# z430/keyword-spotting

Hardware: AMD Instinct MI355X
Metric: 1s 16kHz clips/sec end-to-end (wav->label) (higher is better)
Workload: dtype f32

## Files before the change

### keyword-spotting_amd/csrc/kws_dscnn.hip

```cpp
#include <array>
#include <utility>

#include "kws_dscnn_stages.h"

namespace kws {
namespace {

#ifndef KWS_X_DSCNN_STAMP_TID
#define KWS_X_DSCNN_STAMP_TID 0
#endif

__device__ __forceinline__ DscnnWeights weights_for_this_clip() {
#if defined(__HIP_DEVICE_COMPILE__)
    using KArg = const __attribute__((address_space(4))) DscnnWeights*;
    KArg p = (KArg)__builtin_amdgcn_kernarg_segment_ptr();
    asm volatile("" : "+s"(p));
    return *p;
#else
    return DscnnWeights{};
#endif
}

using FwdKernelFn = void (*)(DscnnWeights, const float*, int, float*, int32_t*, float*, unsigned long long*, const int*, StreamPush);
struct FwdKernelArgs {
// ... 134 lines not shown

    constexpr bool SPLIT = MODE >= 4;
    constexpr bool UT = PERSIST && PAIR;
    BlockTables t1p{};
    uintx4 c1p[PERSIST ? 7 : 1][NP];
    int prev_clip = -1;
    float* a_prev = nullptr;
    if ((MODE == 4 || MODE == 5) && !CLUSTER && tid_k == 0) lds[OFF_ARRIVE] = 0.f;
    if constexpr (PERSIST) {
        fetch_block_tables(w_arg, 1, tid_k, t1p);
        if (wv_k < STAGE_WAVES) stage_features_persist<PAIR, SCAN>(lds, feat, clip, tid_k, sp.scan);
        load_conv1_frags(w_arg, wv_k, lane_k, c1p);
        __syncthreads();
    }
    for (;;) {
    auto weights_now = [&]() -> DscnnWeights { return PERSIST ? weights_for_this_clip() : w_arg; };
    const DscnnWeights w = weights_now();
    int tid = tid_k;
    if constexpr (PERSIST) {
        int wv_l = __builtin_amdgcn_readfirstlane(wv_k), lane_l = lane_k;
        asm volatile("" : "+s"(wv_l), "+v"(lane_l));
        tid = (wv_l << 6) | (lane_l & 63);
    }
    const int lane = tid & 63, wv = tid >> 6;
    if constexpr (PERSIST) n_stamp = 0;
    if (stamps && tid == KWS_X_DSCNN_STAMP_TID) stamps[(size_t)clip * KWS_DSCNN_STAMPS + KWS_DSCNN_STAMPS - 2] = __builtin_amdgcn_s_memrealtime();
    stamp();

    PwOperands<MODE> wa;
    UnitDesc ud{};
    int hops_before = 0;
    int kx = 0, ky[5] = {0, 0, 0, 0, 0}, sg[5] = {0, 0, 0, 0, 0};
    if constexpr (PERSIST) {
        if constexpr (PAIR) {
            const float mxf = read_stage_max(lds, 0, 1);
            kx = pow2_exp_for(mxf);
            const float bz0 = (w.c1_abs * mxf + w.c1_bmax) * 1.001f;
            cap_units(kx, sg[0], w.k_c1, bz0);
            const float by1 = (w.dw_abs[0] * bz0 + w.dw_bmax[0]) * 1.001f;
            ky[1] = pow2_exp_for(by1);
            cap_units(ky[1], sg[1], w.k_pw[0], (w.pw_abs[0] * by1 + w.pw_bmax[0]) * 1.001f);
            store_block_tables(lds, 1, tid, t1p, pow2f(ky[1]), pow2f(sg[1]), pow2f(ky[1] - sg[0]));
            conv1_build_windows(lds, tid, pow2f(kx), OFF_FEAT_P);
            __syncthreads();
        } else {
            store_block_tables(lds, 1, tid, t1p);
        }
        stamp();
        conv1_phase_split<false, NP>(w, lds, tid, c1p, rg0, pow2f(kx), pow2f(sg[0]), OFF_FEAT_P);
        if (wv == NW - 1 && prev_clip >= 0) {
            pool_fc_wave(w, lds, lane, prev_clip, logits, label, a_prev);
            if (stamps && lane == 0) stamps[(size_t)prev_clip * KWS_DSCNN_STAMPS + 13] = __builtin_amdgcn_s_memtime();
        }
        if constexpr (UT) load_unit_desc(w, 1, wv < Leftover<1>::TILE ? wv : Leftover<1>::TILE, lane, ud);
        load_afrag(w, 1, wv >= 4 ? wv - 4 : 0, lane, wa.ring[0]);
    } else if constexpr (PRECONV) {
        static_assert(!PRECONV || MODE >= 4, "the pre-convolved entry exists for the product (split) path only");
        const float* z = feat + (size_t)clip * (CH * P0);
        fetch_block_tables(w, 1, tid, t1_pre);
        float zmax = 0.f;
        for (int i = tid; i < CH * P0; i += NT) {
            const float v = z[i];
            lds[OFF_Z0 + pidx(i / P0, i % P0, P0 + 2)] = v;
            zmax = fmaxf(zmax, v);
        }
        if (tid < CH) {
            lds[OFF_Z0 + pidx(tid, P0, P0 + 2)] = 0.f;
            lds[OFF_Z0 + pidx(tid, P0 + 1, P0 + 2)] = 0.f;
        }
        if constexpr (PAIR)
            publish_wave_max(lds, 1, wv, lane, zmax);
        else
            store_block_tables(lds, 1, tid, t1_pre);
        if constexpr (Leftover<1>::HAS && (MODE == 4 || MODE == 5) && !CLUSTER)
            load_afrag(w, 1, wv >= 4 ? wv - 4 : 0, lane, wa.ring[0]);
        else
            load_block_head(w, 1, lane, wa);
        stamp();
    } else {
    float* featp = lds + OFF_FEAT;
    const float* f = clip_features<SCAN>(feat, clip, sp.scan);
    constexpr int FV = (IN_T * IN_F + NT - 1) / NT;
    float fv[FV];
    int row_new = -1;
    int head;
    if constexpr (STREAM) {
        hops_before = *sp.hops;
        const int K = frames_lag(sp.p);
        head = (((hops_before + 2 - K) % IN_T) + IN_T) % IN_T;
        const int step = sp.p.frame_step;
        const long f_start = (long)step * hops_before + step - (long)K * step;
        if (f_start >= 0) row_new = (int)((((f_start / step) - head) % IN_T + IN_T) % IN_T);
    } else {
        head = ring_hops ? (((*ring_hops + 1 - sp.frames_lag) % IN_T) + IN_T) % IN_T : 0;
    }
#pragma unroll
    for (int k = 0; k < FV; ++k) {
        const int i = tid + k * NT;
        fv[k] = (i < IN_T * IN_F && i / IN_F != row_new) ? f[((i / IN_F + head) % IN_T) * IN_F + i % IN_F] : 0.f;
    }
    BlockTables t1;
    fetch_block_tables(w, 1, tid, t1);
    __builtin_amdgcn_sched_barrier(0);
    float a1[SPLIT ? 1 : 50];
    uintx4 c1f[SPLIT ? 7 : 1][NP];
    if constexpr (SPLIT) {
        load_conv1_frags(w, wv, lane, c1f);
    } else if constexpr (MFMA) {
        const int half = lane >> 5, col = lane & 31, ct = wv & 1;
#pragma unroll
        for (int s = 0; s < 50; ++s) a1[s] = w.c1_w[(2 * s + half) * CH + ct * 32 + col];
        load_pointwise(w, 1, lane, wa);
    }
    __builtin_amdgcn_sched_barrier(0);
    if constexpr (PAIR) {
        float m = 0.f;
#pragma unroll
        for (int k = 0; k < FV; ++k) m = fmaxf(m, fabsf(fv[k]));
        publish_wave_max(lds, 0, wv, lane, m);
    }
    if constexpr (STREAM) {
#ifdef KWS_X_STREAM_NO_FRAME
        if (false)
#else
        if (wv == 0 && cl_tile == cl_n - 1)
#endif
            stream_frame_wave(sp.p, sp.t, sp.hop, clip, clip, false, sp.pcm_ring, sp.ring_len, const_cast<float*>(feat), hops_before,
                              reinterpret_cast<unsigned char*>(lds + OFF_Z2), lane,
                              row_new >= 0 ? featp + (row_new + 2) * FEAT_W + 2 : nullptr, sp.refine_ctr);
        for (int i = tid; i < FEAT_H * FEAT_W; i += NT) {
            const int r = i / FEAT_W - 2, c = i % FEAT_W - 2;
            if (!((unsigned)r < (unsigned)IN_T && (unsigned)c < (unsigned)IN_F)) featp[i] = 0.f;
        }
        if constexpr (!PAIR) store_block_tables(lds, 1, tid, t1);
#pragma unroll
        for (int k = 0; k < FV; ++k) {
            const int i = tid + k * NT;
            if (i < IN_T * IN_F && i / IN_F != row_new) featp[(i / IN_F + 2) * FEAT_W + (i % IN_F) + 2] = fv[k];
        }
        __syncthreads();
    } else {
    for (int i = tid; i < FEAT_H * FEAT_W; i += NT) {
        const int r = i / FEAT_W - 2, c = i % FEAT_W - 2;
        if (!((unsigned)r < (unsigned)IN_T && (unsigned)c < (unsigned)IN_F)) featp[i] = 0.f;
    }
    if constexpr (!PAIR) store_block_tables(lds, 1, tid, t1);
#pragma unroll
    for (int k = 0; k < FV; ++k) {
        const int i = tid + k * NT;
        if (i < IN_T * IN_F) featp[(i / IN_F + 2) * FEAT_W + (i % IN_F) + 2] = fv[k];
    }
    __syncthreads();
    }
    if constexpr (PAIR) {
        float mxf = read_stage_max(lds, 0, 1);
        if constexpr (STREAM) {
            if (row_new >= 0 && cl_tile == cl_n - 1)
                for (int c = 0; c < IN_F; ++c) mxf = fmaxf(mxf, fabsf(featp[(row_new + 2) * FEAT_W + 2 + c]));
        }
        kx = pow2_exp_for(mxf);
        const float bz0 = (w.c1_abs * mxf + w.c1_bmax) * 1.001f;
        cap_units(kx, sg[0], w.k_c1, bz0);
        const float by1 = (w.dw_abs[0] * bz0 + w.dw_bmax[0]) * 1.001f;
        ky[1] = pow2_exp_for(by1);
        cap_units(ky[1], sg[1], w.k_pw[0], (w.pw_abs[0] * by1 + w.pw_bmax[0]) * 1.001f);
        store_block_tables(lds, 1, tid, t1, pow2f(ky[1]), pow2f(sg[1]), pow2f(ky[1] - sg[0]));
        conv1_build_windows(lds, tid, pow2f(kx));
        __syncthreads();
    }
    stamp();

    if constexpr (SPLIT) {
        conv1_phase_split<CLUSTER, NP>(w, lds, tid, c1f, rg0, pow2f(kx), pow2f(sg[0]));
        if constexpr (Leftover<1>::HAS && (MODE == 4 || MODE == 5) && !CLUSTER)
            load_afrag(w, 1, wv >= 4 ? wv - 4 : 0, lane, wa.ring[0]);
        else
            load_block_head(w, 1, lane, wa);
    } else {
        conv1_phase<MFMA>(w, lds, tid, a1);
    }
    }
    stamp();
    const DscnnWeights w1 = weights_now();
    __syncthreads();
    stamp();
    float* a = act ? act + (size_t)clip * KWS_ACT_FLOATS_PER_CLIP : nullptr;
    if (a) {
        const float u = PAIR ? pow2f(-sg[0]) : 1.f;
        for (int i = tid; i < CH * P0; i += NT) a[i] = lds[OFF_Z0 + pidx(i / P0, i % P0, P0 + 2)] * u;
        a += CH * P0;
    }
    PairCtx pc;
    if constexpr (PAIR && PRECONV) {
        const float mz0 = read_stage_max(lds, 1, 1);
        const float by1 = (w1.dw_abs[0] * mz0 + w1.dw_bmax[0]) * 1.001f;
        ky[1] = pow2_exp_for(by1);
        cap_units(ky[1], sg[1], w1.k_pw[0], (w1.pw_abs[0] * by1 + w1.pw_bmax[0]) * 1.001f);
        store_block_tables(lds, 1, tid, t1_pre, pow2f(ky[1]), pow2f(sg[1]), pow2f(ky[1]));
        __syncthreads();
    }
    if constexpr (PAIR) {
        const float mz = read_stage_max(lds, 1, 1) * pow2f(-sg[0]);
        const float bz = (w1.pw_abs[0] * ((w1.dw_abs[0] * mz + w1.dw_bmax[0]) * 1.001f) + w1.pw_bmax[0]) * 1.001f;
        const float by = (w1.dw_abs[1] * bz + w1.dw_bmax[1]) * 1.001f;
        ky[2] = pow2_exp_for(by);
        cap_units(ky[2], sg[2], w1.k_pw[1], (w1.pw_abs[1] * by + w1.pw_bmax[1]) * 1.001f);
        pc.s_dww = pow2f(ky[2] - sg[1]);
        pc.s_dwb = pow2f(ky[2]);
        pc.s_pwb = pow2f(sg[2]);
    }
    block_phase<1, MODE, CLUSTER, UT>(w1, lds, tid, wa, ud, nullptr, rg1, pc);
    stamp();
    const DscnnWeights w2 = weights_now();
    __syncthreads();
    stamp();
    if (a) {
        const float u = PAIR ? pow2f(-sg[1]) : 1.f;
        for (int i = tid; i < CH * Blk<1>::POUT; i += NT)
            a[i] = lds[OFF_Z1 + pidx(i / Blk<1>::POUT, i % Blk<1>::POUT, Blk<1>::SOUT)] * u;
        a += CH * Blk<1>::POUT;
    }
    if constexpr (PAIR) {
        const float mz = fmaxf(read_stage_max(lds, 2, 1) * pow2f(-sg[1]), w2.pw_bmax[0]);
        const float bz = (w2.pw_abs[1] * ((w2.dw_abs[1] * mz + w2.dw_bmax[1]) * 1.001f) + w2.pw_bmax[1]) * 1.001f;
        const float by = (w2.dw_abs[2] * bz + w2.dw_bmax[2]) * 1.001f;
        ky[3] = pow2_exp_for(by);
        cap_units(ky[3], sg[3], w2.k_pw[2], (w2.pw_abs[2] * by + w2.pw_bmax[2]) * 1.001f);
        pc.s_dww = pow2f(ky[3] - sg[2]);
// ... 261 lines not shown
```

### keyword-spotting_amd/csrc/kws_dscnn_geom.h

```cpp
#pragma once
#include "kws_internal.h"

namespace kws {
namespace {

#ifndef KWS_DSCNN_WAVES
#define KWS_DSCNN_WAVES 8
#endif
constexpr int NW = KWS_DSCNN_WAVES;
constexpr int NT = NW * 64;
constexpr int TW = 30;

constexpr int P0 = C1_H * C1_W;
constexpr int FEAT_H = 103, FEAT_W = 14;
constexpr int OFF_Z3 = 0, OFF_Z2 = 22976, OFF_Z1 = 0, OFF_Z0 = 9152, OFF_FEAT = 18304;
constexpr int OFF_DWTAB = 38784;
constexpr int OFF_PWB = OFF_DWTAB + 2 * 768;
constexpr int OFF_POOLED = OFF_PWB + 2 * 64;
constexpr int OFF_POOLBUF = OFF_DWTAB;
constexpr int OFF_WMAX = OFF_POOLED + 64 + 8;
constexpr int OFF_ARRIVE = OFF_WMAX + 3 * NW;
constexpr int LDS_FLOATS = 40960;
static_assert(OFF_ARRIVE + 1 <= LDS_FLOATS, "LDS overflow");
static_assert(NW * 64 <= 768, "pool scratch must fit one depthwise buffer");
static_assert(OFF_FEAT + FEAT_H * FEAT_W <= OFF_Z2, "feature pad overlaps Z2");
static_assert(CH * 12 <= 2 * NT, "table staging assumes at most two elements per thread");

__host__ __device__ __forceinline__ constexpr int pidx(int c, int p, int S) { return (c >> 1) * 2 * S + 2 * p + (c & 1); }

template <int N>
struct Blk {
    static constexpr int H = 45 + 2 * N, W = 1 + 2 * N;
    static constexpr bool RING = N > 1;
    static constexpr int HI = RING ? H - 2 : H, WI = RING ? W - 2 : W;
    static constexpr int PIN = HI * WI, SIN = PIN + 2;
    static constexpr int POUT = H * W, SOUT = POUT + 2;
    static constexpr int OFF_IN = N == 1 ? OFF_Z0 : N == 2 ? OFF_Z1 : N == 3 ? OFF_Z2 : OFF_Z3;
    static constexpr int OFF_OUT = N == 1 ? OFF_Z1 : N == 2 ? OFF_Z2 : OFF_Z3;
    static constexpr int TILES = (POUT + TW - 1) / TW;
    static constexpr int BUF = (N - 1) & 1;
};

#ifndef KWS_DSCNN_KSPLIT_LEFTOVER
#define KWS_DSCNN_KSPLIT_LEFTOVER 1
#endif
template <int N>
struct Leftover {
    static constexpr bool HAS = KWS_DSCNN_KSPLIT_LEFTOVER && (N == 1 || N == 2);
    static constexpr int TILE = N == 1 ? 4 : 8;
    static constexpr int P0T = TILE * TW;
    static constexpr int NP = HAS ? Blk<N>::POUT - P0T : 1;
    static constexpr int WAVE0 = N == 1 ? 4 : 0;
    static constexpr int OFF_PART = N == 1 ? OFF_Z2 : OFF_Z0;
    static constexpr int CSTRIDE = CH + 4;
    static constexpr int PART = NP * CSTRIDE;
};
static_assert(Blk<1>::TILES == 5 && Blk<2>::TILES == 9, "the leftover tiles are the fifth of block 1 and the ninth of block 2");
static_assert(4 * Leftover<1>::PART <= 38784 - OFF_Z2 && OFF_Z0 + 4 * Leftover<2>::PART <= OFF_FEAT, "partial sums fit their dead planes");
static_assert(Leftover<1>::OFF_PART % 4 == 0 && Leftover<2>::OFF_PART % 4 == 0 && Leftover<1>::CSTRIDE % 4 == 0, "partial sums move as float4s");

constexpr int OFF_FEAT_P = OFF_Z2;
constexpr int OFF_POOLBUF_P = OFF_FEAT_P + 1456;
constexpr int STAGE_WAVES = 4;
static_assert(OFF_FEAT_P >= OFF_Z3 + Blk<3>::SOUT * CH, "the next clip's features must not overlap block 4's input");
static_assert(OFF_FEAT_P + FEAT_H * FEAT_W <= OFF_POOLBUF_P && OFF_POOLBUF_P % 4 == 0, "features and pool partials are disjoint");
static_assert(OFF_POOLBUF_P + NW * CH <= OFF_Z2 + Blk<2>::SOUT * CH && OFF_Z2 + Blk<2>::SOUT * CH <= OFF_DWTAB,
              "pool partials stay inside the Z2 plane, clear of the table buffers the next clip's block 1 rewrites");

}
}
```

### keyword-spotting_amd/csrc/kws_dscnn_stages.h

```cpp
#pragma once
#include <type_traits>

#include "kws_dscnn_geom.h"
#include "kws_dscnn_units.h"
#include "kws_mfcc_dev.h"
#include "kws_split_mfma.h"

namespace kws {
namespace {

template <bool TO_MFMA = false>
__device__ __forceinline__ float stencil3x3(float w0, float w1, float w2, float w3, float w4, float w5, float w6,
                                            float w7, float w8, float b, float up, float mid, float dn, float mask_l,
                                            float mask_r) {
    float c, to_right, to_left;
    asm("v_mul_f32 %1, %3, %13\n\t"
        "v_mul_f32 %2, %5, %13\n\t"
        "v_fma_f32 %0, %4, %13, %12\n\t"
        "v_fmac_f32 %1, %6, %14\n\t"
        "v_fmac_f32 %2, %8, %14\n\t"
        "v_fmac_f32 %0, %7, %14\n\t"
        "v_fmac_f32 %1, %9, %15\n\t"
        "v_fmac_f32 %2, %11, %15\n\t"
        "v_fmac_f32 %0, %10, %15\n\t"
// ... 68 lines not shown
    mx = step(mx, std::integral_constant<int, 0x114>{}, std::integral_constant<int, 0xf>{});
    mx = step(mx, std::integral_constant<int, 0x118>{}, std::integral_constant<int, 0xf>{});
    mx = step(mx, std::integral_constant<int, 0x142>{}, std::integral_constant<int, 0xa>{});
    mx = step(mx, std::integral_constant<int, 0x143>{}, std::integral_constant<int, 0xc>{});
    if (lane == 63) lds[OFF_WMAX + set * NW + wv] = mx;
}
__device__ __forceinline__ float read_stage_max(const float* lds, int set0, int n_sets) {
    static_assert(NW % 4 == 0 && OFF_WMAX % 4 == 0, "the stage maxima are read as float4s");
    float m = 0.f;
    const float4* q = reinterpret_cast<const float4*>(lds + OFF_WMAX + set0 * NW);
    for (int i = 0; i < (NW / 4) * n_sets; ++i) {
        const float4 v = q[i];
        m = fmaxf(fmaxf(m, fmaxf(v.x, v.y)), fmaxf(v.z, v.w));
    }
    return m;
}

template <int NP>
struct PwRing {
    uintx4 ring[2][2][NP];
};
struct PwRegsF32 {
    float wa[2][32];
};
template <int MODE>
using PwOperands = std::conditional_t<(MODE >= 4), PwRing<(MODE == 5 ? 2 : 3)>, PwRegsF32>;
__device__ __forceinline__ void load_pointwise(const DscnnWeights& w, int n, int lane, PwRegsF32& o) {
    const float* pw = w.pw_w + (n - 1) * CH * CH + 8 * (lane >> 5) * CH + (lane & 31);
#pragma unroll
    for (int ct = 0; ct < 2; ++ct)
#pragma unroll
        for (int s = 0; s < 32; ++s) o.wa[ct][s] = pw[(16 * (s >> 3) + (s & 7)) * CH + ct * 32];
}
template <int NP>
__device__ __forceinline__ void load_afrag(const DscnnWeights& w, int n, int m, int lane, uintx4 (&f)[2][NP]) {
    const uintx4* src = reinterpret_cast<const uintx4*>(NP == 2 ? w.pw_pair : w.pw_split) + (size_t)(n - 1) * (2 * 4 * NP * 64) + lane;
#pragma unroll
    for (int ct = 0; ct < 2; ++ct)
#pragma unroll
        for (int p = 0; p < NP; ++p) f[ct][p] = src[((ct * 4 + m) * NP + p) * 64];
}
__device__ __forceinline__ void load_block_head(const DscnnWeights& w, int n, int lane, PwRegsF32& o) { load_pointwise(w, n, lane, o); }
template <int NP>
__device__ __forceinline__ void load_block_head(const DscnnWeights& w, int n, int lane, PwRing<NP>& o) { load_afrag(w, n, 0, lane, o.ring[0]); }

struct UnitDesc {
    uintx4 a;
    uint2 m;
};
__device__ __forceinline__ void load_unit_desc(const DscnnWeights& w, int n, int tile, int lane, UnitDesc& d) {
    const uint32_t* src = w.units + ((size_t)(ds_unit_base(n - 1) + tile) * 2 * 64 + lane) * 4;
    d.a = *reinterpret_cast<const uintx4*>(src);
    d.m = *reinterpret_cast<const uint2*>(src + 64 * 4);
}

template <bool MFMA>
__device__ __forceinline__ void conv1_phase(const DscnnWeights& w, float* lds, int tid, const float (&a)[50]) {
    const float* featp = lds + OFF_FEAT;
    float* z0 = lds + OFF_Z0;
    if constexpr (MFMA) {
        const int lane = tid & 63, wv = tid >> 6, half = lane >> 5, col = lane & 31;
        const int ct = wv & 1;
        for (int u = wv; u < 10; u += NW) {
            const int pt = u >> 1;
            const int pos = pt * 32 + col;
            const int posc = pos < P0 ? pos : P0 - 1;
            const int oh = posc / C1_W, ow = posc % C1_W;
            const float* base = featp + (2 * oh) * FEAT_W + 2 * ow + half;
            floatx16 acc = {0, 0, 0, 0, 0, 0, 0, 0, 0, 0, 0, 0, 0, 0, 0, 0};
#pragma unroll
            for (int s = 0; s < 50; ++s) {
                const float b = base[((2 * s) / 10) * FEAT_W + (2 * s) % 10];
                acc = __builtin_amdgcn_mfma_f32_32x32x2f32(a[s], b, acc, 0, 0, 0);
            }
            if (pos < P0) {
#pragma unroll
                for (int r = 0; r < 16; ++r) {
                    const int co = ct * 32 + row_of(r, half);
                    z0[pidx(co, pos, P0 + 2)] = relu(acc[r] + w.c1_b[co]);
                }
            }
        }
    } else {
        for (int idx = tid; idx < CH * P0; idx += NT) {
            const int co = idx / P0, pos = idx % P0;
            const int oh = pos / C1_W, ow = pos % C1_W;
            float acc = w.c1_b[co];
            for (int kh = 0; kh < C1_K; ++kh)
                for (int kw = 0; kw < C1_K; ++kw)
                    acc = fmaf(w.c1_w[(kh * C1_K + kw) * CH + co], featp[(2 * oh + kh) * FEAT_W + 2 * ow + kw], acc);
            z0[pidx(co, pos, P0 + 2)] = relu(acc);
        }
    }
    if (tid < CH) {
        z0[pidx(tid, P0, P0 + 2)] = 0.f;
        z0[pidx(tid, P0 + 1, P0 + 2)] = 0.f;
    }
}

template <bool DUAL, int NP>
__device__ __forceinline__ void conv1_unit_split(const DscnnWeights& w, const float* featp, float* z0, int ptile, int ct, int lane,
                                                 const uintx4 (&c1f)[7][NP], int p_lo, int p_hi, float sx, float sig0, float& mx) {
    constexpr bool PAIR = NP == 2;
    const int half = lane >> 5, col = lane & 31;
    const int pos = p_lo + ptile * 32 + col;
    const int posc = pos < p_hi ? pos : p_hi - 1;
// ... 210 lines not shown
        for (int r = 0; r < 16; r += 2) {
            const int co = ct * 32 + row_of(r, half);
            const float4 b4 = cb[r >> 2];
            const float b0 = (r & 2) ? b4.z : b4.x, b1 = (r & 2) ? b4.w : b4.y;
            const float v0 = relu(fmaf(b0, sig0, acc[r])), v1 = relu(fmaf(b1, sig0, acc[r + 1]));
            *reinterpret_cast<float2*>(z0 + pidx(co, pos, P0 + 2)) = make_float2(v0, v1);
            mx = fmaxf(mx, fmaxf(v0, v1));
            if (DUAL) {
                const int oo = (ct ^ 1) * 32 + row_of(r, half);
                const float4 o4 = ob[DUAL ? (r >> 2) : 0];
                const float c0 = (r & 2) ? o4.z : o4.x, c1 = (r & 2) ? o4.w : o4.y;
                const float u0 = relu(fmaf(c0, sig0, occ[r])), u1 = relu(fmaf(c1, sig0, occ[r + 1]));
                *reinterpret_cast<float2*>(z0 + pidx(oo, pos, P0 + 2)) = make_float2(u0, u1);
                mx = fmaxf(mx, fmaxf(u0, u1));
            }
        }
    }
}

struct PosRange {
    int lo, hi;
};

template <bool RANGED, int NP>
__device__ __forceinline__ void conv1_phase_split(const DscnnWeights& w, float* lds, int tid, const uintx4 (&c1f)[7][NP],
                                                  PosRange rg, float sx = 1.f, float sig0 = 1.f, int off_feat = OFF_FEAT) {
    static_assert(P0 > 4 * 32 && P0 <= 5 * 32 && NW >= 6, "conv1 work split: four dual tiles + one tile in two halves");
    const float* featp = lds + off_feat;
    float* z0 = lds + OFF_Z0;
    const int lane = tid & 63, wv = tid >> 6;
    float mx = 0.f;
    if constexpr (NP == 2) {
        if constexpr (RANGED) {
            const int n_pt = (rg.hi - rg.lo + 31) / 32;
            for (int u = wv; u < 2 * n_pt; u += NW) conv1_unit_pairwin<false>(w, lds, z0, u >> 1, u & 1, lane, c1f, rg.lo, rg.hi, sig0, mx);
        } else if (wv < 4)
            conv1_unit_pairwin<true>(w, lds, z0, wv, wv & 1, lane, c1f, 0, P0, sig0, mx);
        else if (wv < 6)
            conv1_unit_pairwin<false>(w, lds, z0, 4, wv & 1, lane, c1f, 0, P0, sig0, mx);
    } else if constexpr (RANGED) {
        const int n_pt = (rg.hi - rg.lo + 31) / 32;
        for (int u = wv; u < 2 * n_pt; u += NW) conv1_unit_split<false, NP>(w, featp, z0, u >> 1, u & 1, lane, c1f, rg.lo, rg.hi, sx, sig0, mx);
    } else if (wv < 4)
        conv1_unit_split<true, NP>(w, featp, z0, wv, wv & 1, lane, c1f, 0, P0, sx, sig0, mx);
    else if (wv < 6)
        conv1_unit_split<false, NP>(w, featp, z0, 4, wv & 1, lane, c1f, 0, P0, sx, sig0, mx);
    if constexpr (NP == 2) publish_wave_max(lds, 1, wv, lane, mx);
    if (tid < CH) {
        z0[pidx(tid, P0, P0 + 2)] = 0.f;
        z0[pidx(tid, P0 + 1, P0 + 2)] = 0.f;
    }
}

template <int N, int NP, bool UT = false>
__device__ __forceinline__ void leftover_partial_unit(float* lds, int lane, int M, const uintx4 (&af)[2][NP], const UnitDesc& ud) {
    using G = Blk<N>;
    using L = Leftover<N>;
    const int half = lane >> 5, col = lane & 31;
    const float* dwtab = lds + OFF_DWTAB + G::BUF * 768;
    const float4* dwt4 = reinterpret_cast<const float4*>(dwtab) + half * 24;
    bool valid;
    float mask_l, mask_r;
    int ta[3];
    if constexpr (UT) {
        valid = ud.a[3] != 0u;
        mask_l = __builtin_bit_cast(float, ud.m.x), mask_r = __builtin_bit_cast(float, ud.m.y);
#pragma unroll
        for (int i = 0; i < 3; ++i) ta[i] = (int)ud.a[i];
    } else {
        const int pos = L::P0T - 1 + col;
        valid = col >= 1 && col <= TW && pos < G::POUT;
        const int posc = pos < G::POUT ? pos : G::POUT - 1;
        const int h = posc / G::W, x = posc % G::W;
        mask_l = x > 0 ? 1.f : 0.f, mask_r = x < G::W - 1 ? 1.f : 0.f;
#pragma unroll
        for (int dh = -1; dh <= 1; ++dh) {
            const int o = G::RING ? 1 : 0;
            const int hh = h + dh - o, xx = x - o;
            const bool inside = (unsigned)hh < (unsigned)G::HI && (unsigned)xx < (unsigned)G::WI;
            const bool in_map = (unsigned)(h + dh) < (unsigned)G::H;
            const int a = inside ? hh * G::WI + xx : ((G::RING && in_map) ? G::PIN : G::PIN + 1);
            ta[dh + 1] = G::OFF_IN + pidx(half * 8, a, G::SIN);
        }
    }
    float y[8];
#pragma unroll
    for (int j = 0; j < 8; j += 2) {
        const int cs = 16 * M + j;
        const int o = cs * G::SIN;
        const float2 up = *reinterpret_cast<const float2*>(lds + ta[0] + o);
        const float2 mid = *reinterpret_cast<const float2*>(lds + ta[1] + o);
        const float2 dn = *reinterpret_cast<const float2*>(lds + ta[2] + o);
        DwPair wp;
#pragma unroll
        for (int i = 0; i < 5; ++i) wp.l[i] = dwt4[(cs >> 1) * 6 + i];
        y[j] = stencil3x3_of_pair<false, 0>(wp, up.x, mid.x, dn.x, mask_l, mask_r);
        y[j + 1] = stencil3x3_of_pair<false, 1>(wp, up.y, mid.y, dn.y, mask_l, mask_r);
    }
    floatx16 acc0 = {0, 0, 0, 0, 0, 0, 0, 0, 0, 0, 0, 0, 0, 0, 0, 0}, acc1 = acc0;
    if constexpr (NP == 2) {
        uintx4 bh, bl;
        split_pair8_scaled(y, bh, bl);
        acc0 = mfma_f16(af[0][0], bl, acc0);
        acc1 = mfma_f16(af[1][0], bl, acc1);
        acc0 = mfma_f16(af[0][1], bh, acc0);
        acc1 = mfma_f16(af[1][1], bh, acc1);
        acc0 = mfma_f16(af[0][0], bh, acc0);
        acc1 = mfma_f16(af[1][0], bh, acc1);
    } else {
        uintx4 bh, bm, bl;
        split3(y, bh, bm, bl);
#pragma unroll
        for (int q = 0; q < 6; ++q) {
            const int pa = q == 0 ? 2 : (q == 2 || q == 3) ? 1 : 0;
            const uintx4& b = (q == 0 || q == 3 || q == 5) ? bh : (q == 1 ? bl : bm);
            acc0 = mfma_bf16(af[0][pa], b, acc0);
            acc1 = mfma_bf16(af[1][pa], b, acc1);
        }
    }
    if (valid) {
        float4* part4 = reinterpret_cast<float4*>(lds + L::OFF_PART + M * L::PART + (col - 1) * L::CSTRIDE) + half;
#pragma unroll
        for (int q = 0; q < 4; ++q) {
            part4[2 * q] = make_float4(acc0[4 * q], acc0[4 * q + 1], acc0[4 * q + 2], acc0[4 * q + 3]);
            part4[8 + 2 * q] = make_float4(acc1[4 * q], acc1[4 * q + 1], acc1[4 * q + 2], acc1[4 * q + 3]);
        }
    }
}

template <int N>
__device__ __forceinline__ float leftover_arrive(float* lds, int lane) {
    using G = Blk<N>;
    using L = Leftover<N>;
    int* arrived = reinterpret_cast<int*>(lds + OFF_ARRIVE);
    asm volatile("s_waitcnt lgkmcnt(0)" ::: "memory");
    int before = 0;
    if (lane == 0) before = __hip_atomic_fetch_add(arrived, 1, __ATOMIC_RELAXED, __HIP_MEMORY_SCOPE_WORKGROUP);
    before = __builtin_amdgcn_readfirstlane(before);
    asm volatile("" ::: "memory");
    float mx = 0.f;
    if (before == 3) {
        const float4* part4 = reinterpret_cast<const float4*>(lds + L::OFF_PART);
        float* zout = lds + G::OFF_OUT;
        const int cq = lane & 15;
        const float4 b = reinterpret_cast<const float4*>(lds + OFF_PWB + G::BUF * 64)[cq];
        constexpr int ROUNDS = (L::NP + 3) / 4, RB = 2;
        static_assert(ROUNDS % RB == 0, "whole batches");
        auto comb = [&](float p0, float p1, float p2, float p3, float bias) { return relu(((p0 + p1) + (p2 + p3)) + bias); };
#pragma unroll 1
        for (int r0 = 0; r0 < ROUNDS; r0 += RB) {
            float4 p[RB][4];
// ... 17 lines not shown
                }
            }
        }
        if (lane == 0) *arrived = 0;
    }
    return mx;
}

template <int N, int MODE, bool RANGED = false, bool UT = false>
__device__ __forceinline__ void block_phase(const DscnnWeights& w, float* lds, int tid, PwOperands<MODE>& pwo, UnitDesc& ud,
                                            float* __restrict__ act4 = nullptr, PosRange rg = PosRange{0, 0}, PairCtx pc = PairCtx{},
                                            int off_poolbuf = OFF_POOLBUF) {
    static_assert(!UT || ((MODE == 4 || MODE == 5) && !RANGED && Leftover<1>::HAS), "unit descriptors: product paths on whole maps");
    using G = Blk<N>;
    constexpr bool PAIR = MODE == 5;
    constexpr int NP = PAIR ? 2 : 3;
    constexpr int NPROD = PAIR ? 3 : 6;
    constexpr bool KSL = Leftover<N>::HAS && (MODE == 4 || MODE == 5) && !RANGED;
    const int p_lo = RANGED ? rg.lo : 0, p_hi = RANGED ? rg.hi : G::POUT;
#ifdef KWS_X_DSCNN_SKIP_LEFTOVER
    const int n_tiles = RANGED ? (p_hi - p_lo + TW - 1) / TW : (N == 2 ? 8 : G::TILES);
#else
    const int n_tiles = RANGED ? (p_hi - p_lo + TW - 1) / TW : (KSL ? Leftover<N>::TILE : G::TILES);
#endif
    constexpr bool MFMA = MODE != 0;
    constexpr bool SPLIT = MODE >= 4;
    constexpr bool NO_STENCIL = MODE == 6;
    const int lane = tid & 63, wv = tid >> 6, half = lane >> 5, col = lane & 31;
    float* zout = lds + G::OFF_OUT;
    const float* dwtab = lds + OFF_DWTAB + G::BUF * 768;
    const float* pwb = lds + OFF_PWB + G::BUF * 64;
    float* poolbuf = lds + off_poolbuf;

    BlockTables next_tables;
    if constexpr (N < 4) {
        fetch_block_tables(w, N + 1, tid, next_tables);
        if (tid < CH) {
            zout[pidx(tid, G::POUT, G::SOUT)] = relu(pwb[tid]);
            zout[pidx(tid, G::POUT + 1, G::SOUT)] = 0.f;
        }
    } else if (!MFMA) {
        poolbuf[wv * CH + lane] = 0.f;
    }

    const float4* bias4 = reinterpret_cast<const float4*>(pwb) + half;
    const float4* dwt4 = reinterpret_cast<const float4*>(dwtab) + half * 24;
    float psum[2][16];
#pragma unroll
    for (int ct = 0; ct < 2; ++ct)
#pragma unroll
        for (int r = 0; r < 16; ++r) psum[ct][r] = 0.f;
    float stage_max = 0.f;

    for (int t = wv; t < n_tiles; t += NW) {
        const int pos = p_lo + t * TW - 1 + col;
        bool valid;
        uint32_t keep;
        float mask_l, mask_r;
        int tlo[3], thi[3];
        if constexpr (UT) {
            keep = ud.a[3];
            valid = keep != 0u;
            mask_l = __builtin_bit_cast(float, ud.m.x), mask_r = __builtin_bit_cast(float, ud.m.y);
#pragma unroll
            for (int i = 0; i < 3; ++i) {
                tlo[i] = (int)ud.a[i];
                thi[i] = tlo[i] + 32 * G::SIN;
                asm volatile("" : "+v"(tlo[i]));
                asm volatile("" : "+v"(thi[i]));
            }
        } else {
            valid = col >= 1 && col <= TW && pos < p_hi;
            keep = valid ? 0xffffffffu : 0u;
            const int posc = pos < p_lo ? p_lo : (pos < p_hi ? pos : p_hi - 1);
            const int h = posc / G::W, x = posc % G::W;
            mask_l = x > 0 ? 1.f : 0.f, mask_r = x < G::W - 1 ? 1.f : 0.f;
#pragma unroll
            for (int dh = -1; dh <= 1; ++dh) {
                const int o = G::RING ? 1 : 0;
                const int hh = h + dh - o, xx = x - o;
                const bool inside = (unsigned)hh < (unsigned)G::HI && (unsigned)xx < (unsigned)G::WI;
                const bool in_map = (unsigned)(h + dh) < (unsigned)G::H;
                const int a = inside ? hh * G::WI + xx : ((G::RING && in_map) ? G::PIN : G::PIN + 1);
                tlo[dh + 1] = G::OFF_IN + pidx(half * 8, a, G::SIN);
                thi[dh + 1] = tlo[dh + 1] + 32 * G::SIN;
                asm volatile("" : "+v"(tlo[dh + 1]));
                asm volatile("" : "+v"(thi[dh + 1]));
            }
        }
        UnitDesc ud_next = ud;

        auto cs_of = [](int s) { return 16 * (s >> 3) + (s & 7); };
        struct TapPair {
            float2 up, mid, dn;
        };
        auto tap_pair_load = [&](int sp, TapPair& tp) {
            const int cs = cs_of(2 * sp);
            const int* ta = cs < 32 ? tlo : thi;
            const int o = (cs & 31) * G::SIN;
            if constexpr (!NO_STENCIL) {
                tp.up = *reinterpret_cast<const float2*>(lds + ta[0] + o);
                tp.dn = *reinterpret_cast<const float2*>(lds + ta[2] + o);
            }
            tp.mid = *reinterpret_cast<const float2*>(lds + ta[1] + o);
        };
        auto wts_pair_load = [&](int sp, DwPair& wp) {
            const int cs = cs_of(2 * sp);
// ... 15 lines not shown
            }
            DwPair wq0, wq1;
            TapPair tq0, tq1;
            if constexpr (!NO_STENCIL) {
                wts_pair_load(0, wq0);
                wts_pair_load(1, wq1);
            }
            tap_pair_load(0, tq0);
            tap_pair_load(1, tq1);
            __builtin_amdgcn_sched_barrier(0);
            if constexpr (SPLIT) {
                float y[8];
                uintx4 bh, bm, bl;
                auto product = [&](int ct, int m, int q) {
                    const int pa = PAIR ? (q == 1 ? 1 : 0) : (q == 0 ? 2 : (q == 2 || q == 3) ? 1 : 0);
                    const uintx4& b = PAIR ? (q == 0 ? bl : bh) : ((q == 0 || q == 3 || q == 5) ? bh : (q == 1 ? bl : bm));
                    if constexpr (PAIR) {
                        if (ct == 0)
                            acc0 = mfma_f16(pwo.ring[m & 1][0][pa], b, acc0);
                        else
                            acc1 = mfma_f16(pwo.ring[m & 1][1][pa], b, acc1);
                    } else {
                        if (ct == 0)
                            acc0 = mfma_bf16(pwo.ring[m & 1][0][pa], b, acc0);
                        else
                            acc1 = mfma_bf16(pwo.ring[m & 1][1][pa], b, acc1);
                    }
                    __builtin_amdgcn_sched_barrier(0);
                };
#pragma unroll
                for (int s = 0; s < 32; ++s) {
                    const int m = s >> 3, j = s & 7;
                    DwPair& wp = (s & 2) ? wq1 : wq0;
                    TapPair& tq = (s & 2) ? tq1 : tq0;
                    const bool feed = m > 0 && j < NPROD;
                    if (feed) product(0, m - 1, j);
                    if constexpr (NO_STENCIL)
                        y[j] = (s & 1) ? tq.mid.y : tq.mid.x;
                    else
                        y[j] = (s & 1) ? dw_eval(wp, tq, std::integral_constant<int, 1>{}) : dw_eval(wp, tq, std::integral_constant<int, 0>{});
                    __builtin_amdgcn_sched_barrier(0);
                    if (feed) product(1, m - 1, j);
                    if ((s & 1) && s + 3 < 32) {
                        if constexpr (!NO_STENCIL) wts_pair_load((s >> 1) + 2, wp);
                        tap_pair_load((s >> 1) + 2, tq);
                    }
                    __builtin_amdgcn_sched_barrier(0);
                    if (j == 6) {
                        if (m < 3) {
                            load_afrag(w, N, m + 1, lane, pwo.ring[(m + 1) & 1]);
                        } else if (t + NW < n_tiles) {
                            if constexpr (UT) load_unit_desc(w, N, t + NW, lane, ud_next);
                            load_afrag(w, N, 0, lane, pwo.ring[0]);
                        } else if (KSL && N == 2 && wv < 4) {
                            if constexpr (UT) load_unit_desc(w, N, Leftover<N>::TILE, lane, ud_next);
                            load_afrag(w, N, wv, lane, pwo.ring[0]);
                        } else if (N < 4) {
                            if constexpr (UT) load_unit_desc(w, N < 4 ? N + 1 : N, wv, lane, ud_next);
                            load_afrag(w, N < 4 ? N + 1 : N, 0, lane, pwo.ring[0]);
                        }
                        __builtin_amdgcn_sched_barrier(0);
                    }
                    if (j == 7) {
                        if constexpr (PAIR) {
                            split_pair8_scaled(y, bh, bl);
                        } else {
                            split3(y, bh, bm, bl);
                        }
                        __builtin_amdgcn_sched_barrier(0);
                    }
                }
#pragma unroll
                for (int q = 0; q < NPROD; ++q) {
                    product(0, 3, q);
                    product(1, 3, q);
                }
            } else {
                auto& wa = pwo.wa;
#pragma unroll
                for (int s = 0; s < 32; s += 2) {
                    TapPair& tq = (s & 2) ? tq1 : tq0;
                    DwPair& wp = (s & 2) ? wq1 : wq0;
                    float y0, y1;
                    if constexpr (MODE == 2) {
                        y0 = tq.mid.x;
                        y1 = tq.mid.y;
                    } else {
                        y0 = dw_eval(wp, tq, std::integral_constant<int, 0>{});
                        y1 = dw_eval(wp, tq, std::integral_constant<int, 1>{});
                        if (s + 4 < 32) {
                            wts_pair_load((s >> 1) + 2, wp);
                            tap_pair_load((s >> 1) + 2, tq);
                        }
                        __builtin_amdgcn_sched_barrier(0);
                    }
                    if constexpr (MODE == 3) {
                        acc0[0] += y0 * wa[0][s];
                        acc1[0] += y1 * wa[1][s + 1];
                    } else {
                        acc0 = __builtin_amdgcn_mfma_f32_32x32x2f32(wa[0][s], y0, acc0, 0, 0, 0);
                        acc1 = __builtin_amdgcn_mfma_f32_32x32x2f32(wa[1][s], y0, acc1, 0, 0, 0);
                        acc0 = __builtin_amdgcn_mfma_f32_32x32x2f32(wa[0][s + 1], y1, acc0, 0, 0, 0);
                        acc1 = __builtin_amdgcn_mfma_f32_32x32x2f32(wa[1][s + 1], y1, acc1, 0, 0, 0);
                    }
                }
            }
            auto epilogue = [&]() {
#ifndef KWS_X_NO_MFMA_EPILOGUE_NOP
                asm volatile("s_nop 15\n\ts_nop 3" : "+v"(acc0), "+v"(acc1));
#endif
                if constexpr (N < 4) {
                    if constexpr (PAIR && N <= 2) {
// ... 28 lines not shown
                        psum[1][r] += __builtin_bit_cast(float, __builtin_bit_cast(uint32_t, relu(acc1[r])) & keep);
                    }
                    if (act4 && valid) {
#pragma unroll
                        for (int r = 0; r < 16; ++r) {
                            act4[row_of(r, half) * G::POUT + pos] = relu(acc0[r]) * pc.inv_out;
                            act4[(32 + row_of(r, half)) * G::POUT + pos] = relu(acc1[r]) * pc.inv_out;
                        }
                    }
                }
            };
            if constexpr (!SPLIT) {
                if (N < 4 && t + NW >= n_tiles) {
                    __builtin_amdgcn_sched_barrier(0);
                    if constexpr (N < 4) load_pointwise(w, N + 1, lane, pwo);
                    __builtin_amdgcn_sched_barrier(0);
                    epilogue();
                    break;
                }
            }
            epilogue();
            if constexpr (UT) ud = ud_next;
        } else {
            const float* pw_w = w.pw_w + (N - 1) * CH * CH;
            float y[32];
#pragma unroll
            for (int s = 0; s < 32; s += 2) {
                TapPair tq;
                tap_pair_load(s >> 1, tq);
                DwPair wp;
                wts_pair_load(s >> 1, wp);
                y[s] = dw_eval(wp, tq, std::integral_constant<int, 0>{});
                y[s + 1] = dw_eval(wp, tq, std::integral_constant<int, 1>{});
            }
#pragma unroll 1
            for (int co = 0; co < CH; ++co) {
                float part = 0.f;
#pragma unroll
                for (int s = 0; s < 32; ++s) part = fmaf(pw_w[(16 * (s >> 3) + 8 * half + (s & 7)) * CH + co], y[s], part);
                const float tot = relu(part + __shfl_xor(part, 32, 64) + pwb[co]);
                if constexpr (N < 4) {
                    if (valid && half == 0) zout[pidx(co, pos, G::SOUT)] = tot;
                } else {
                    if (act4 && valid && half == 0) act4[co * G::POUT + pos] = tot;
                    float sum = (valid && half == 0) ? tot : 0.f;
#pragma unroll
                    for (int o = 16; o >= 1; o >>= 1) sum += __shfl_xor(sum, o, 64);
                    if (lane == 0) poolbuf[wv * CH + co] += sum;
                }
            }
        }
    }

    if constexpr (KSL) {
        using L = Leftover<N>;
        if (wv >= L::WAVE0 && wv < L::WAVE0 + 4) {
            leftover_partial_unit<N, NP, UT>(lds, lane, wv - L::WAVE0, pwo.ring[0], ud);
            __builtin_amdgcn_sched_barrier(0);
            if constexpr (UT) load_unit_desc(w, N + 1, wv, lane, ud);
            load_afrag(w, N + 1, 0, lane, pwo.ring[0]);
            __builtin_amdgcn_sched_barrier(0);
            stage_max = fmaxf(stage_max, leftover_arrive<N>(lds, lane));
        }
    }
    if constexpr (N < 4) store_block_tables(lds, N + 1, tid, next_tables, pc.s_dwb, pc.s_pwb, pc.s_dww);
    if constexpr (PAIR && N <= 2) publish_wave_max(lds, N == 1 ? 2 : 0, wv, lane, stage_max);
    if constexpr (MFMA) {
        if constexpr (N < 4) {
            if (wv >= n_tiles && !(KSL && N == 1)) load_block_head(w, N + 1, lane, pwo);
        } else {
#pragma unroll
            for (int ct = 0; ct < 2; ++ct) {
                float (&q)[16] = psum[ct];
                asm volatile("s_nop 4\n\t"
                    "v_add_f32_dpp %0, %0, %0 row_shr:1 row_mask:0xf bank_mask:0xf bound_ctrl:1\n\t"
                    "v_add_f32_dpp %1, %1, %1 row_shr:1 row_mask:0xf bank_mask:0xf bound_ctrl:1\n\t"
                    "v_add_f32_dpp %2, %2, %2 row_shr:1 row_mask:0xf bank_mask:0xf bound_ctrl:1\n\t"
                    "v_add_f32_dpp %3, %3, %3 row_shr:1 row_mask:0xf bank_mask:0xf bound_ctrl:1\n\t"
                    "v_add_f32_dpp %4, %4, %4 row_shr:1 row_mask:0xf bank_mask:0xf bound_ctrl:1\n\t"
                    "v_add_f32_dpp %5, %5, %5 row_shr:1 row_mask:0xf bank_mask:0xf bound_ctrl:1\n\t"
                    "v_add_f32_dpp %6, %6, %6 row_shr:1 row_mask:0xf bank_mask:0xf bound_ctrl:1\n\t"
                    "v_add_f32_dpp %7, %7, %7 row_shr:1 row_mask:0xf bank_mask:0xf bound_ctrl:1\n\t"
                    "v_add_f32_dpp %8, %8, %8 row_shr:1 row_mask:0xf bank_mask:0xf bound_ctrl:1\n\t"
                    "v_add_f32_dpp %9, %9, %9 row_shr:1 row_mask:0xf bank_mask:0xf bound_ctrl:1\n\t"
                    "v_add_f32_dpp %10, %10, %10 row_shr:1 row_mask:0xf bank_mask:0xf bound_ctrl:1\n\t"
                    "v_add_f32_dpp %11, %11, %11 row_shr:1 row_mask:0xf bank_mask:0xf bound_ctrl:1\n\t"
                    "v_add_f32_dpp %12, %12, %12 row_shr:1 row_mask:0xf bank_mask:0xf bound_ctrl:1\n\t"
                    "v_add_f32_dpp %13, %13, %13 row_shr:1 row_mask:0xf bank_mask:0xf bound_ctrl:1\n\t"
                    "v_add_f32_dpp %14, %14, %14 row_shr:1 row_mask:0xf bank_mask:0xf bound_ctrl:1\n\t"
                    "v_add_f32_dpp %15, %15, %15 row_shr:1 row_mask:0xf bank_mask:0xf bound_ctrl:1\n\t"
                    "v_add_f32_dpp %0, %0, %0 row_shr:2 row_mask:0xf bank_mask:0xf bound_ctrl:1\n\t"
                    "v_add_f32_dpp %1, %1, %1 row_shr:2 row_mask:0xf bank_mask:0xf bound_ctrl:1\n\t"
                    "v_add_f32_dpp %2, %2, %2 row_shr:2 row_mask:0xf bank_mask:0xf bound_ctrl:1\n\t"
                    "v_add_f32_dpp %3, %3, %3 row_shr:2 row_mask:0xf bank_mask:0xf bound_ctrl:1\n\t"
                    "v_add_f32_dpp %4, %4, %4 row_shr:2 row_mask:0xf bank_mask:0xf bound_ctrl:1\n\t"
                    "v_add_f32_dpp %5, %5, %5 row_shr:2 row_mask:0xf bank_mask:0xf bound_ctrl:1\n\t"
                    "v_add_f32_dpp %6, %6, %6 row_shr:2 row_mask:0xf bank_mask:0xf bound_ctrl:1\n\t"
                    "v_add_f32_dpp %7, %7, %7 row_shr:2 row_mask:0xf bank_mask:0xf bound_ctrl:1\n\t"
                    "v_add_f32_dpp %8, %8, %8 row_shr:2 row_mask:0xf bank_mask:0xf bound_ctrl:1\n\t"
                    "v_add_f32_dpp %9, %9, %9 row_shr:2 row_mask:0xf bank_mask:0xf bound_ctrl:1\n\t"
                    "v_add_f32_dpp %10, %10, %10 row_shr:2 row_mask:0xf bank_mask:0xf bound_ctrl:1\n\t"
                    "v_add_f32_dpp %11, %11, %11 row_shr:2 row_mask:0xf bank_mask:0xf bound_ctrl:1\n\t"
                    "v_add_f32_dpp %12, %12, %12 row_shr:2 row_mask:0xf bank_mask:0xf bound_ctrl:1\n\t"
                    "v_add_f32_dpp %13, %13, %13 row_shr:2 row_mask:0xf bank_mask:0xf bound_ctrl:1\n\t"
                    "v_add_f32_dpp %14, %14, %14 row_shr:2 row_mask:0xf bank_mask:0xf bound_ctrl:1\n\t"
                    "v_add_f32_dpp %15, %15, %15 row_shr:2 row_mask:0xf bank_mask:0xf bound_ctrl:1\n\t"
                    "v_add_f32_dpp %0, %0, %0 row_shr:4 row_mask:0xf bank_mask:0xf bound_ctrl:1\n\t"
                    "v_add_f32_dpp %1, %1, %1 row_shr:4 row_mask:0xf bank_mask:0xf bound_ctrl:1\n\t"
                    "v_add_f32_dpp %2, %2, %2 row_shr:4 row_mask:0xf bank_mask:0xf bound_ctrl:1\n\t"
                    "v_add_f32_dpp %3, %3, %3 row_shr:4 row_mask:0xf bank_mask:0xf bound_ctrl:1\n\t"
                    "v_add_f32_dpp %4, %4, %4 row_shr:4 row_mask:0xf bank_mask:0xf bound_ctrl:1\n\t"
                    "v_add_f32_dpp %5, %5, %5 row_shr:4 row_mask:0xf bank_mask:0xf bound_ctrl:1\n\t"
                    "v_add_f32_dpp %6, %6, %6 row_shr:4 row_mask:0xf bank_mask:0xf bound_ctrl:1\n\t"
                    "v_add_f32_dpp %7, %7, %7 row_shr:4 row_mask:0xf bank_mask:0xf bound_ctrl:1\n\t"
                    "v_add_f32_dpp %8, %8, %8 row_shr:4 row_mask:0xf bank_mask:0xf bound_ctrl:1\n\t"
                    "v_add_f32_dpp %9, %9, %9 row_shr:4 row_mask:0xf bank_mask:0xf bound_ctrl:1\n\t"
                    "v_add_f32_dpp %10, %10, %10 row_shr:4 row_mask:0xf bank_mask:0xf bound_ctrl:1\n\t"
// ... 73 lines not shown
```

Before: 7.468 million.

## Run leftover K-split quarter before regular tiles in blocks one and two

Reorders per-wave work in depthwise-separable blocks 1 and 2 so the waves owning the leftover K-split quarter do that partial unit first, then their regular tiles, instead of after the tile loop. A new request_first_unit helper picks the right tile and k-block for each wave's first prefetch, and a callback in leftover_partial_unit issues the next unit-descriptor load once the stencil taps are done. The aim is to shorten the critical path of the partial-sum arrival and balance wave finish times ahead of the stage barrier. It changes the tile-to-wave mapping for block 1 and adds prefetch bookkeeping that must stay consistent, with a compile-time flag to fall back.

```diff
diff --git a/keyword-spotting_amd/csrc/kws_dscnn.hip b/keyword-spotting_amd/csrc/kws_dscnn.hip
--- a/keyword-spotting_amd/csrc/kws_dscnn.hip
+++ b/keyword-spotting_amd/csrc/kws_dscnn.hip
@@ -210,8 +210,7 @@
             pool_fc_wave(w, lds, lane, prev_clip, logits, label, a_prev);
             if (stamps && lane == 0) stamps[(size_t)prev_clip * KWS_DSCNN_STAMPS + 13] = __builtin_amdgcn_s_memtime();
         }
-        if constexpr (UT) load_unit_desc(w, 1, wv < Leftover<1>::TILE ? wv : Leftover<1>::TILE, lane, ud);
-        load_afrag(w, 1, wv >= 4 ? wv - 4 : 0, lane, wa.ring[0]);
+        request_first_unit<1, true, UT>(w, wv, lane, ud, wa.ring[0]);
     } else if constexpr (PRECONV) {
         static_assert(!PRECONV || MODE >= 4, "the pre-convolved entry exists for the product (split) path only");
         const float* z = feat + (size_t)clip * (CH * P0);
@@ -231,7 +230,7 @@
         else
             store_block_tables(lds, 1, tid, t1_pre);
         if constexpr (Leftover<1>::HAS && (MODE == 4 || MODE == 5) && !CLUSTER)
-            load_afrag(w, 1, wv >= 4 ? wv - 4 : 0, lane, wa.ring[0]);
+            request_first_unit<1, true, false>(w, wv, lane, ud, wa.ring[0]);
         else
             load_block_head(w, 1, lane, wa);
         stamp();
@@ -331,7 +330,7 @@
     if constexpr (SPLIT) {
         conv1_phase_split<CLUSTER, NP>(w, lds, tid, c1f, rg0, pow2f(kx), pow2f(sg[0]));
         if constexpr (Leftover<1>::HAS && (MODE == 4 || MODE == 5) && !CLUSTER)
-            load_afrag(w, 1, wv >= 4 ? wv - 4 : 0, lane, wa.ring[0]);
+            request_first_unit<1, true, false>(w, wv, lane, ud, wa.ring[0]);
         else
             load_block_head(w, 1, lane, wa);
     } else {
diff --git a/keyword-spotting_amd/csrc/kws_dscnn_geom.h b/keyword-spotting_amd/csrc/kws_dscnn_geom.h
--- a/keyword-spotting_amd/csrc/kws_dscnn_geom.h
+++ b/keyword-spotting_amd/csrc/kws_dscnn_geom.h
@@ -44,6 +44,9 @@
 #ifndef KWS_DSCNN_KSPLIT_LEFTOVER
 #define KWS_DSCNN_KSPLIT_LEFTOVER 1
 #endif
+#ifndef KWS_DSCNN_B2_QUARTER_FIRST
+#define KWS_DSCNN_B2_QUARTER_FIRST 1
+#endif
 template <int N>
 struct Leftover {
     static constexpr bool HAS = KWS_DSCNN_KSPLIT_LEFTOVER && (N == 1 || N == 2);
@@ -51,6 +54,8 @@
     static constexpr int P0T = TILE * TW;
     static constexpr int NP = HAS ? Blk<N>::POUT - P0T : 1;
     static constexpr int WAVE0 = N == 1 ? 4 : 0;
+    static constexpr int TILE_WAVE0 = N == 1 ? 4 - WAVE0 : 0;
+    static constexpr bool THEN_TILE = N == 2 && KWS_DSCNN_B2_QUARTER_FIRST;
     static constexpr int OFF_PART = N == 1 ? OFF_Z2 : OFF_Z0;
     static constexpr int CSTRIDE = CH + 4;
     static constexpr int PART = NP * CSTRIDE;
diff --git a/keyword-spotting_amd/csrc/kws_dscnn_stages.h b/keyword-spotting_amd/csrc/kws_dscnn_stages.h
--- a/keyword-spotting_amd/csrc/kws_dscnn_stages.h
+++ b/keyword-spotting_amd/csrc/kws_dscnn_stages.h
@@ -144,6 +144,23 @@
     const uint32_t* src = w.units + ((size_t)(ds_unit_base(n - 1) + tile) * 2 * 64 + lane) * 4;
     d.a = *reinterpret_cast<const uintx4*>(src);
     d.m = *reinterpret_cast<const uint2*>(src + 64 * 4);
+}
+template <int N, bool KSL, bool UT, int NP>
+__device__ __forceinline__ void request_first_unit(const DscnnWeights& w, int wv, int lane, UnitDesc& ud, uintx4 (&ring0)[2][NP]) {
+    using L = Leftover<N>;
+    int tile = wv, kb = 0;
+    if constexpr (KSL && L::HAS) {
+        const bool quarter = wv >= L::WAVE0 && wv < L::WAVE0 + 4;
+        if (N == 1) {
+            tile = quarter ? L::TILE : wv - L::TILE_WAVE0;
+            kb = quarter ? wv - L::WAVE0 : 0;
+        } else if (L::THEN_TILE && quarter) {
+            tile = L::TILE;
+            kb = wv - L::WAVE0;
+        }
+    }
+    if constexpr (UT) load_unit_desc(w, N, tile, lane, ud);
+    load_afrag(w, N, kb, lane, ring0);
 }
 
 template <bool MFMA>
@@ -460,8 +477,8 @@
     }
 }
 
-template <int N, int NP, bool UT = false>
-__device__ __forceinline__ void leftover_partial_unit(float* lds, int lane, int M, const uintx4 (&af)[2][NP], const UnitDesc& ud) {
+template <int N, int NP, bool UT = false, class F>
+__device__ __forceinline__ void leftover_partial_unit(float* lds, int lane, int M, const uintx4 (&af)[2][NP], const UnitDesc& ud, F&& taps_done) {
     using G = Blk<N>;
     using L = Leftover<N>;
     const int half = lane >> 5, col = lane & 31;
@@ -505,6 +522,7 @@
         y[j] = stencil3x3_of_pair<false, 0>(wp, up.x, mid.x, dn.x, mask_l, mask_r);
         y[j + 1] = stencil3x3_of_pair<false, 1>(wp, up.y, mid.y, dn.y, mask_l, mask_r);
     }
+    taps_done();
     floatx16 acc0 = {0, 0, 0, 0, 0, 0, 0, 0, 0, 0, 0, 0, 0, 0, 0, 0}, acc1 = acc0;
     if constexpr (NP == 2) {
         uintx4 bh, bl;
@@ -628,7 +646,32 @@
         for (int r = 0; r < 16; ++r) psum[ct][r] = 0.f;
     float stage_max = 0.f;
 
-    for (int t = wv; t < n_tiles; t += NW) {
+    auto leftover_quarter = [&]() {
+        if constexpr (KSL) {
+            using L = Leftover<N>;
+            leftover_partial_unit<N, NP, UT>(lds, lane, wv - L::WAVE0, pwo.ring[0], ud, [&]() {
+                if constexpr (L::THEN_TILE && UT) {
+                    __builtin_amdgcn_sched_barrier(0);
+                    load_unit_desc(w, N, wv - L::TILE_WAVE0, lane, ud);
+                    __builtin_amdgcn_sched_barrier(0);
+                }
+            });
+            __builtin_amdgcn_sched_barrier(0);
+            if constexpr (L::THEN_TILE)
+                load_afrag(w, N, 0, lane, pwo.ring[0]);
+            else
+                request_first_unit<N + 1, KSL, UT>(w, wv, lane, ud, pwo.ring[0]);
+            __builtin_amdgcn_sched_barrier(0);
+            stage_max = fmaxf(stage_max, leftover_arrive<N>(lds, lane));
+        }
+    };
+    constexpr bool QUARTER_FIRST = KSL && (N == 1 || Leftover<N>::THEN_TILE);
+    const bool quarter_wave = KSL && wv >= Leftover<N>::WAVE0 && wv < Leftover<N>::WAVE0 + 4;
+    if constexpr (QUARTER_FIRST)
+        if (quarter_wave) leftover_quarter();
+
+    const int t_first = KSL && N == 1 ? (quarter_wave ? n_tiles : wv - Leftover<N>::TILE_WAVE0) : wv;
+    for (int t = t_first; t < n_tiles; t += NW) {
         const int pos = p_lo + t * TW - 1 + col;
         bool valid;
         uint32_t keep;
@@ -750,12 +793,11 @@
                         } else if (t + NW < n_tiles) {
                             if constexpr (UT) load_unit_desc(w, N, t + NW, lane, ud_next);
                             load_afrag(w, N, 0, lane, pwo.ring[0]);
-                        } else if (KSL && N == 2 && wv < 4) {
+                        } else if (KSL && N == 2 && !Leftover<N>::THEN_TILE && wv < 4) {
                             if constexpr (UT) load_unit_desc(w, N, Leftover<N>::TILE, lane, ud_next);
                             load_afrag(w, N, wv, lane, pwo.ring[0]);
                         } else if (N < 4) {
-                            if constexpr (UT) load_unit_desc(w, N < 4 ? N + 1 : N, wv, lane, ud_next);
-                            load_afrag(w, N < 4 ? N + 1 : N, 0, lane, pwo.ring[0]);
+                            request_first_unit<(N < 4 ? N + 1 : N), KSL, UT>(w, wv, lane, ud_next, pwo.ring[0]);
                         }
                         __builtin_amdgcn_sched_barrier(0);
                     }
@@ -890,17 +932,8 @@
         }
     }
 
-    if constexpr (KSL) {
-        using L = Leftover<N>;
-        if (wv >= L::WAVE0 && wv < L::WAVE0 + 4) {
-            leftover_partial_unit<N, NP, UT>(lds, lane, wv - L::WAVE0, pwo.ring[0], ud);
-            __builtin_amdgcn_sched_barrier(0);
-            if constexpr (UT) load_unit_desc(w, N + 1, wv, lane, ud);
-            load_afrag(w, N + 1, 0, lane, pwo.ring[0]);
-            __builtin_amdgcn_sched_barrier(0);
-            stage_max = fmaxf(stage_max, leftover_arrive<N>(lds, lane));
-        }
-    }
+    if constexpr (KSL && !QUARTER_FIRST)
+        if (quarter_wave) leftover_quarter();
     if constexpr (N < 4) store_block_tables(lds, N + 1, tid, next_tables, pc.s_dwb, pc.s_pwb, pc.s_dww);
     if constexpr (PAIR && N <= 2) publish_wave_max(lds, N == 1 ? 2 : 0, wv, lane, stage_max);
     if constexpr (MFMA) {
```

Result: no change. 7.496 million, median of 6 (+0.4%).
